# syoyo/lucille

Hardware: AMD Instinct MI355X
Metric: Mrays/s (primary+AO) (higher is better)
Workload: dtype f32 filter + f64 resolve (hit records f64); 1 GPU; S-soup-1M ray dump (BASELINE config 3): 1000000 random triangles, one dump of 100000000 incoherent rays cut into 1 contiguous slice(s), closest-hit; rays=100000000, rays_per_gpu=100000000, triangles=1000000, mode=closest, variant=-1, parallelism=replicated BVH, ray slices x1

## Files before the change

lucille_amd/csrc/lh_device.h:

```cpp
#ifndef LH_DEVICE_H
#define LH_DEVICE_H

#include <stdint.h>
#include <stddef.h>
#include "../../include/lucille_hip.h"

#define LH_BLOCK      256
#define LH_MISS_PRIM  0xFFFFFFFFu
#define LH_T_INF      1.0e38

typedef struct lh_dev_scene {
    const void *nodes;
    const void *tri32;
    const void *tri64;
    float       grid_lo[3], grid_step[3];
    const void *q4nodes;
    uint32_t    nq4nodes, q4_depth;
    uint32_t    q4_stack;
    const void *q8nodes;
    uint32_t    nq8nodes, q8_depth;
    int         prefer_q8;
    uint32_t    stack_rows;
    const void *ref_lca;
    const void *prim_leafpos;
    const void *ref_nodes;
    const void *ref_leaf_prims;
    uint32_t    ref_nnodes;
    int         ref_empty;
    double      ref_bmin[3], ref_bmax[3];
    uint32_t    ntris;
    uint32_t    nnodes;
    uint32_t    max_depth;
    float       scene_r;
    float       deg_dcap;
    uint32_t    cap_srcs;
    uint32_t    ndanger;
    uint32_t    danger[3];
    uint32_t    ray_chunk;
    uint32_t    ray_budget;
    int         stack_guard;
    uint32_t    stack_cap;
    uint32_t    coop_patience;
    uint32_t    ao_group;
    uint32_t    top_nodes;
    uint32_t    io_fmt;
    const void *cam_src;
    const uint32_t *n_dev;
    uint32_t   *diag_out;
    unsigned long long *diag_clock;
} lh_dev_scene_t;

enum { LH_CNT_NODES = 0, LH_CNT_TRIS = 1, LH_CNT_EXACT = 2, LH_CNT_RAYS = 3, LH_CNT_N = 4,
       LH_CNT_NODE_SLOTS = 4, LH_CNT_TRI_SLOTS = 5, LH_CNT_REGROUP_SLOTS = 6,
       LH_CNT_RETRACED = 7,
       LH_CNT_HIST = 8,
       LH_CNT_DEV = 32 };

enum {
    LH_VARIANT_DIRECT = 0,
    LH_VARIANT_SPEC   = 4
};

#define LH_ROWS_UNCHECKED 64u
#define LH_TOP_AUTO       0xFFFFFFFFu
#define LH_TOP_NODES_MAX  512u
#define LH_ROWS_CHECKED   34u
#define LH_NPART          8
#define LH_CURSOR_STRIDE  32
#define LH_CURSOR_WORDS   ((LH_NPART + 1) * LH_CURSOR_STRIDE)
#define LH_AO_QCAP        (1u << 22)
#define LH_DUMP_BUDGET    2048u
#define LH_DUMP_MIN_ACTIVE 24
#define LH_DUMP_TRI_BATCH  8
#define LH_DUMP8_MIN_ACTIVE 40
#define LH_DUMP8_TRI_BATCH  20
#define LH_TILE_CHUNK     1024u
#define LH_AO_BUDGET      384u
#define LH_RAY_BUDGET     128u
#define LH_PRIM_OVERFLOW  0xFFFFFFFDu
#define LH_OCC_OVERFLOW   4u
#define LH_IO_RAYS_F32    1u
#define LH_IO_REC16       2u

#ifdef __cplusplus
extern "C" {
#endif

typedef struct lh_fixq {
    void     *queue;
    uint32_t *qcount;
    uint32_t  qcap;
    void     *aux_stream;
    void     *ev_ready, *ev_done;
} lh_fixq_t;

int lh_launch_trace(const lh_dev_scene_t *sc, size_t n, const double *d_org,
                    const double *d_dir, uint32_t *d_prim, double *d_t,
                    double *d_u, double *d_v, int anyhit, uint8_t *d_occluded,
                    unsigned long long *d_counters ,
                    unsigned long long *d_workq ,
                    int variant, int grid_blocks, int min_active, int tri_batch,
                    const lh_fixq_t *q, int ncus, void *stream);
int lh_launch_trace_ao(const lh_dev_scene_t *sc, size_t nslots, int ntheta, int nphi, unsigned long long seed,
                       const double *d_hitrec, const unsigned long long *d_slot_key, unsigned int *d_occ_count,
                       unsigned long long *d_counters, unsigned long long *d_cursor, int grid_blocks, int min_active,
                       int tri_batch, const lh_fixq_t *q, int ncus, const unsigned long long *d_nslots, uint32_t budget_big, void *stream);
int lh_trace_formats_needed(const lh_dev_scene_t *sc, int variant);
int lh_trace_rows(const lh_dev_scene_t *sc);

// ... 5 lines not shown
```

lucille_amd/csrc/lh_filter.h:

```cpp
#ifndef LH_FILTER_H
#define LH_FILTER_H

#include <math.h>
#include <stdint.h>

#if defined(__HIPCC__)
#define LH_HD __host__ __device__ __forceinline__
#else
#define LH_HD static inline
#endif

#if defined(__HIP_DEVICE_COMPILE__)
#define LH_RCP(a) __builtin_amdgcn_rcpf(a)
#else
#define LH_RCP(a) (1.0f / (a))
#endif

#define LH_EPS24 5.9604645e-8f
#define LH_KBOX  16.0f
#define LH_KTRI  32.0f

typedef struct lh_ray32 {
    float ox, oy, oz, dx, dy, dz;
    float ix, iy, iz;
// ... 29 lines not shown
LH_HD void lh_ray_setup(lh_ray32_t *r, double ox, double oy, double oz,
                        double dx, double dy, double dz, float scene_r)
{
    float omax, scale, pe, sx, sy, sz;
    r->ox = (float)ox; r->oy = (float)oy; r->oz = (float)oz;
    r->dx = (float)dx; r->dy = (float)dy; r->dz = (float)dz;
    r->ix = 1.0f / lh_safe_dir(r->dx);
    r->iy = 1.0f / lh_safe_dir(r->dy);
    r->iz = 1.0f / lh_safe_dir(r->dz);
    omax = fmaxf(fabsf(r->ox), fmaxf(fabsf(r->oy), fabsf(r->oz)));
    scale = omax + scene_r;
    pe = LH_KBOX * LH_EPS24 * scale;
    sx = pe * fabsf(r->ix); sy = pe * fabsf(r->iy); sz = pe * fabsf(r->iz);
    r->cnx = fmaf(-r->ox, r->ix, -sx); r->cfx = fmaf(-r->ox, r->ix, sx);
    r->cny = fmaf(-r->oy, r->iy, -sy); r->cfy = fmaf(-r->oy, r->iy, sy);
    r->cnz = fmaf(-r->oz, r->iz, -sz); r->cfz = fmaf(-r->oz, r->iz, sz);
    r->ngx = r->dx < 0.0f; r->ngy = r->dy < 0.0f; r->ngz = r->dz < 0.0f;
    r->keps = LH_KTRI * LH_EPS24 * scale;
    r->qax = r->qay = r->qaz = 0.0f; r->qbnx = r->qbny = r->qbnz = 0.0f; r->qbfx = r->qbfy = r->qbfz = 0.0f;
    r->dn = sqrtf(fmaf(r->dx, r->dx, fmaf(r->dy, r->dy, r->dz * r->dz))) * 1.000001f;
}

LH_HD int lh_slab(const lh_ray32_t *r, float lox, float loy, float loz,
                  float hix, float hiy, float hiz, float tb, float *tn_out)
{
    const float ax = r->ngx ? hix : lox, bx = r->ngx ? lox : hix;
    const float ay = r->ngy ? hiy : loy, by = r->ngy ? loy : hiy;
    const float az = r->ngz ? hiz : loz, bz = r->ngz ? loz : hiz;
    const float tn = fmaxf(fmaxf(fmaf(ax, r->ix, r->cnx), fmaf(ay, r->iy, r->cny)),
                           fmaxf(fmaf(az, r->iz, r->cnz), 0.0f));
    const float tf = fminf(fminf(fmaf(bx, r->ix, r->cfx), fmaf(by, r->iy, r->cfy)),
                           fminf(fmaf(bz, r->iz, r->cfz), tb));
    *tn_out = tn;
    return tn <= tf;
}

LH_HD int lh_slab_w(const lh_ray32_t *r, uint32_t wx, uint32_t wy, uint32_t wz, float tb, float *tn_out)
{
    const uint32_t sx = r->ngx ? ((wx >> 16) | (wx << 16)) : wx;
    const uint32_t sy = r->ngy ? ((wy >> 16) | (wy << 16)) : wy;
    const uint32_t sz = r->ngz ? ((wz >> 16) | (wz << 16)) : wz;
    const float tn = fmaxf(fmaxf(fmaf((float)(sx & 0xffffu), r->qax, r->qbnx), fmaf((float)(sy & 0xffffu), r->qay, r->qbny)),
                           fmaxf(fmaf((float)(sz & 0xffffu), r->qaz, r->qbnz), 0.0f));
    const float tf = fminf(fminf(fmaf((float)(sx >> 16), r->qax, r->qbfx), fmaf((float)(sy >> 16), r->qay, r->qbfy)),
                           fminf(fmaf((float)(sz >> 16), r->qaz, r->qbfz), tb));
    *tn_out = tn;
    return tn <= tf;
}

#define LH_TRI_REJECT    0
#define LH_TRI_CANDIDATE 1
#define LH_TRI_CERTAIN   2

LH_HD int lh_tri_filter(const lh_ray32_t *r, float v0x, float v0y, float v0z,
                        float e1x, float e1y, float e1z, float e2x, float e2y, float e2z,
                        float ne1, float ne2, float tb, float *t_hi)
{
    const float px = fmaf(r->dy, e2z, -(r->dz * e2y));
    const float py = fmaf(r->dz, e2x, -(r->dx * e2z));
    const float pz = fmaf(r->dx, e2y, -(r->dy * e2x));
    const float a = fmaf(e1x, px, fmaf(e1y, py, e1z * pz));
    const float inva = LH_RCP(a);
    const float sx = r->ox - v0x, sy = r->oy - v0y, sz = r->oz - v0z;
    const float qx = fmaf(sy, e1z, -(sz * e1y));
    const float qy = fmaf(sz, e1x, -(sx * e1z));
    const float qz = fmaf(sx, e1y, -(sy * e1x));
    const float u = fmaf(sx, px, fmaf(sy, py, sz * pz)) * inva;
    const float v = fmaf(qx, r->dx, fmaf(qy, r->dy, qz * r->dz)) * inva;
    const float t = fmaf(e2x, qx, fmaf(e2y, qy, e2z * qz)) * inva;
    const float g = r->keps * fabsf(inva);
    const float tolu = g * r->dn * ne2, tolv = g * r->dn * ne1, tolt = g * ne1 * ne2;
    const float rela = (LH_KTRI * LH_EPS24) * ne1 * ne2 * r->dn * fabsf(inva);
    if (!(rela < 0.5f)) { *t_hi = 3.0e38f; return LH_TRI_CANDIDATE; }
    const int reject = (u < -tolu) | (u > 1.0f + tolu) | (v < -tolv) |
                       (u + v > 1.0f + tolu + tolv) | (t < -tolt) | (t - tolt > tb);
    if (reject) return LH_TRI_REJECT;
    {
        const int sure = (u >= tolu) & (u <= 1.0f - tolu) & (v >= tolv) &
                         (u + v <= 1.0f - tolu - tolv) & (t >= tolt) & (rela < 0.25f) &
                         (fabsf(a) > 2.0e-14f) & (t + tolt < 1.0e37f);
        *t_hi = (t + tolt) * 1.000001f;
        return sure ? LH_TRI_CERTAIN : LH_TRI_CANDIDATE;
    }
}

#if defined(__clang__)
#define LH_NO_CONTRACT _Pragma("clang fp contract(off)")
#else
#define LH_NO_CONTRACT
#endif

LH_HD int lh_exact_isect(const double *tv, double ox, double oy, double oz,
                         double dx, double dy, double dz,
                         double *t_out, double *u_out, double *v_out)
{
    LH_NO_CONTRACT
    const double v0x = tv[0], v0y = tv[1], v0z = tv[2];
    const double e1x = tv[3] - v0x, e1y = tv[4] - v0y, e1z = tv[5] - v0z;
    const double e2x = tv[6] - v0x, e2y = tv[7] - v0y, e2z = tv[8] - v0z;
    const double px = dy * e2z - dz * e2y;
    const double py = dz * e2x - dx * e2z;
    const double pz = dx * e2y - dy * e2x;
    const double a = e1x * px + e1y * py + e1z * pz;
    double inva, sx, sy, sz, qx, qy, qz, u, v, t;
    if (!(fabs(a) > 1.0e-14)) return 0;
    inva = 1.0 / a;
    sx = ox - v0x; sy = oy - v0y; sz = oz - v0z;
    qx = sy * e1z - sz * e1y;
    qy = sz * e1x - sx * e1z;
    qz = sx * e1y - sy * e1x;
    u = (sx * px + sy * py + sz * pz) * inva;
    v = (qx * dx + qy * dy + qz * dz) * inva;
    t = (e2x * qx + e2y * qy + e2z * qz) * inva;
    if ((u < 0.0) || (u > 1.0)) return 0;
    if ((v < 0.0) || ((u + v) > 1.0)) return 0;
    if (t < 0.0) return 0;
    *t_out = t; *u_out = u; *v_out = v;
    return 1;
}

#endif
```

lucille_amd/csrc/lh_kernels.hip:

```cpp
#include <hip/hip_runtime.h>
#include <stdint.h>
#include <string.h>
#include <stdlib.h>
#include <pthread.h>

#include "../../include/lucille_hip.h"
#include "lh_device.h"
#include "lh_filter.h"
#include "lh_reftrace.h"
#include "lh_ao.h"

namespace {

#include "lh_walk.h"
#include "lh_pt.h"

template <bool ANYHIT, bool COUNT>
__device__ __forceinline__ void traverse(Lane &L, const lh_dev_scene_t &sc,
                                         int (*stk)[LH_BLOCK], const int tid,
                                         double ox, double oy, double oz,
                                         double dx, double dy, double dz, Best &best,
                                         uint32_t &c_nodes, uint32_t &c_tris, uint32_t &c_exact)
{
    const float4 *__restrict__ tris  = (const float4 *)sc.tri32;
// ... 62 lines not shown
    const int base = L.sp + nh - 1;
    if (SORTED) {
        const uint32_t k0 = h0 ? ((__float_as_uint(t0) & ~3u) | 0u) : 0xFFFFFFFCu;
        const uint32_t k1 = h1 ? ((__float_as_uint(t1) & ~3u) | 1u) : 0xFFFFFFFDu;
        const uint32_t k2 = h2 ? ((__float_as_uint(t2) & ~3u) | 2u) : 0xFFFFFFFEu;
        const uint32_t k3 = h3 ? ((__float_as_uint(t3) & ~3u) | 3u) : 0xFFFFFFFFu;
        const int b10 = k1 < k0, b20 = k2 < k0, b30 = k3 < k0, b21 = k2 < k1, b31 = k3 < k1, b32 = k3 < k2;
        const int rk0 = b10 + b20 + b30, rk1 = (1 - b10) + b21 + b31;
        const int rk2 = (2 - b20 - b21) + b32, rk3 = 3 - b30 - b31 - b32;
        stk[LH_ROW(h0 ? base - rk0 : L.sp + rk0)][tid] = (int)r.x;
        stk[LH_ROW(h1 ? base - rk1 : L.sp + rk1)][tid] = (int)r.y;
        stk[LH_ROW(h2 ? base - rk2 : L.sp + rk2)][tid] = (int)r.z;
        stk[LH_ROW(h3 ? base - rk3 : L.sp + rk3)][tid] = (int)r.w;
    } else {
        const int a1 = (int)h0, a2 = a1 + (int)h1, a3 = a2 + (int)h2;
        stk[LH_ROW(h0 ? base : base + 1)][tid] = (int)r.x;
        stk[LH_ROW(h1 ? base - a1 : base + 1)][tid] = (int)r.y;
        stk[LH_ROW(h2 ? base - a2 : base + 1)][tid] = (int)r.z;
        stk[LH_ROW(h3 ? base - a3 : base + 1)][tid] = (int)r.w;
    }
    L.sp = base;
    const int nxt = stk[LH_ROW(base)][tid];
    const int popped2 = stk[LH_ROW(L.sp - 1)][tid];
    const bool is_leaf = (nxt < 0) & (nxt != kDone);
    const bool park = is_leaf & (pend == kNoLeaf);
    pend = park ? nxt : pend;
    L.cur = park ? popped2 : nxt;
    L.sp -= park ? 1 : 0;
}

template <bool ANYHIT, bool COUNT, int STRIDE, bool RING>
__device__ __forceinline__ void tri_pass(Lane &L, int &pend, const lh_dev_scene_t &sc, int (*stk)[STRIDE], const int tid,
                                         double ox, double oy, double oz, double dx, double dy, double dz, Best &best,
                                         uint32_t &c_tris, uint32_t &c_exact, const int ring_mask = 0)
{
    if (pend != kNoLeaf) {
        const float4 *__restrict__ tris = (const float4 *)sc.tri32;
        const uint32_t x = ~(uint32_t)pend;
        const float4 *tp = tris + 3 * (size_t)(x >> 2);
        const float4 ta = tp[0], tb_ = tp[1], tc = tp[2];
        if (COUNT) c_tris++;
        const bool finished = tri_step<ANYHIT, COUNT>(L, sc, ta.x, ta.y, ta.z, ta.w, tb_.x, tb_.y, tb_.z, tb_.w, tc.x, tc.z, tc.w, __float_as_uint(tc.y), ox, oy, oz, dx, dy, dz, best, c_exact);
        if (finished) { L.cur = kDone; pend = kNoLeaf; }
        else if (x & 3u) pend = (int)~(((x >> 2) + 1u) << 2 | ((x & 3u) - 1u));
        else {
            const bool waiting = (L.cur < 0) & (L.cur != kDone);
            pend = waiting ? L.cur : kNoLeaf;
            if (waiting) { L.sp--; L.cur = stk[LH_ROW(L.sp)][tid]; }
        }
    }
#undef LH_ROW
}

template <bool ANYHIT, bool COUNT, bool GUARD, bool SORTED = true>
__device__ __forceinline__ void traverse_spec4(Lane &L, int &pend, const lh_dev_scene_t &sc,
                                               int (*stk)[LH_BLOCK], const int tid,
                                               double ox, double oy, double oz,
                                               double dx, double dy, double dz, Best &best,
                                               uint32_t &c_nodes, uint32_t &c_tris, uint32_t &c_exact,
                                               const int min_active, const int tri_batch,
                                               uint32_t &c_nslots, uint32_t &c_tslots, uint32_t &it)
{
    const int rows = (int)sc.stack_rows;
    const uint4 *top = (const uint4 *)(&stk[rows][0]);
    const uint32_t ntop = sc.top_nodes;
    for (;;) {
        if (COUNT) { if (__ballot(L.cur >= 0) != 0ull) c_nslots++; }
        if (GUARD) {
            const bool ov = (L.cur >= 0) & (L.sp + 4 > rows);
            if (__builtin_expect(__ballot(ov) != 0ull, 0)) { if (ov) { L.over = true; L.cur = kDone; pend = kNoLeaf; } }
        }
        if (L.cur >= 0) node_step4<COUNT, LH_BLOCK, false, SORTED>(L, pend, sc, stk, tid, c_nodes, 0, top, ntop);
        const unsigned long long m_node = __ballot(L.cur >= 0);
        const unsigned long long m_pend = __ballot(pend != kNoLeaf);
        if (m_pend != 0ull && (__popcll(m_pend) >= tri_batch || m_node == 0ull)) {
            if (COUNT) c_tslots++;
            tri_pass<ANYHIT, COUNT, LH_BLOCK, false>(L, pend, sc, stk, tid, ox, oy, oz, dx, dy, dz, best, c_tris, c_exact);
        }
        const unsigned long long m_work = __ballot((L.cur != kDone) | (pend != kNoLeaf));
        if (__popcll(m_work) < min_active || (++it & kRegroupMask) == 0u) break;
    }
}

template <bool ANYHIT, bool COUNT>
__device__ __forceinline__ void traverse_spec8(Lane &L, int &pend, const lh_dev_scene_t &sc,
                                               int (*stk)[LH_BLOCK], const int tid,
                                               double ox, double oy, double oz,
                                               double dx, double dy, double dz, Best &best,
                                               uint32_t &c_nodes, uint32_t &c_tris, uint32_t &c_exact,
                                               const int min_active, const int tri_batch,
                                               uint32_t &c_nslots, uint32_t &c_tslots, uint32_t &it)
{
    const float4 *__restrict__ tris  = (const float4 *)sc.tri32;
    const uint32_t oct = (uint32_t)L.r.ngx | ((uint32_t)L.r.ngy << 1) | ((uint32_t)L.r.ngz << 2);
    const int rows = (int)sc.stack_rows - 1;

    for (;;) {
        if (COUNT) { if (__ballot(L.cur >= 0) != 0ull) c_nslots++; }
        if (sc.stack_guard && L.cur >= 0 && L.sp + 8 > rows) { L.over = true; L.cur = kDone; pend = kNoLeaf; }
        if (L.cur >= 0) {
            const uint4 *p = (const uint4 *)sc.q8nodes + 8 * (size_t)L.cur;
            const uint4 a = p[0], b = p[1], c = p[2], d = p[3], e = p[4], f = p[5], r0 = p[6], r1 = p[7];
            if (COUNT) c_nodes++;
            float t;
            const bool h0 = slab_w(L, a.x, a.y, a.z, t) & ((int)r0.x != kDone);
            const bool h1 = slab_w(L, a.w, b.x, b.y, t) & ((int)r0.y != kDone);
            const bool h2 = slab_w(L, b.z, b.w, c.x, t) & ((int)r0.z != kDone);
            const bool h3 = slab_w(L, c.y, c.z, c.w, t) & ((int)r0.w != kDone);
            const bool h4 = slab_w(L, d.x, d.y, d.z, t) & ((int)r1.x != kDone);
            const bool h5 = slab_w(L, d.w, e.x, e.y, t) & ((int)r1.y != kDone);
            const bool h6 = slab_w(L, e.z, e.w, f.x, t) & ((int)r1.z != kDone);
            const bool h7 = slab_w(L, f.y, f.z, f.w, t) & ((int)r1.w != kDone);
            const uint32_t pm = ((uint32_t)h0 << (0u ^ oct)) | ((uint32_t)h1 << (1u ^ oct)) | ((uint32_t)h2 << (2u ^ oct)) |
                                ((uint32_t)h3 << (3u ^ oct)) | ((uint32_t)h4 << (4u ^ oct)) | ((uint32_t)h5 << (5u ^ oct)) |
                                ((uint32_t)h6 << (6u ^ oct)) | ((uint32_t)h7 << (7u ^ oct));
            const int base = L.sp + __popc(pm) - 1;
#define LH_PUSH8(S, H, REF) stk[(H) ? base - __popc(pm & ((1u << ((S) ^ oct)) - 1u)) : rows][tid] = (int)(REF)
            LH_PUSH8(0u, h0, r0.x); LH_PUSH8(1u, h1, r0.y); LH_PUSH8(2u, h2, r0.z); LH_PUSH8(3u, h3, r0.w);
            LH_PUSH8(4u, h4, r1.x); LH_PUSH8(5u, h5, r1.y); LH_PUSH8(6u, h6, r1.z); LH_PUSH8(7u, h7, r1.w);
#undef LH_PUSH8
            L.sp = base;
            const int nxt = stk[base][tid];
            const int popped2 = stk[L.sp - 1][tid];
            const bool is_leaf = (nxt < 0) & (nxt != kDone);
            const bool park = is_leaf & (pend == kNoLeaf);
            pend = park ? nxt : pend;
            L.cur = park ? popped2 : nxt;
            L.sp -= park ? 1 : 0;
        }
        const unsigned long long m_node = __ballot(L.cur >= 0);
        const unsigned long long m_pend = __ballot(pend != kNoLeaf);
        if (m_pend != 0ull && (__popcll(m_pend) >= tri_batch || m_node == 0ull)) {
            if (COUNT) c_tslots++;
            if (pend != kNoLeaf) {
                const uint32_t x = ~(uint32_t)pend;
                const float4 *tp = tris + 3 * (size_t)(x >> 2);
                const float4 ta = tp[0], tb_ = tp[1], tc = tp[2];
                if (COUNT) c_tris++;
                const bool finished = tri_step<ANYHIT, COUNT>(L, sc, ta.x, ta.y, ta.z, ta.w, tb_.x, tb_.y, tb_.z, tb_.w, tc.x, tc.z, tc.w, __float_as_uint(tc.y), ox, oy, oz, dx, dy, dz, best, c_exact);
                if (finished) { L.cur = kDone; pend = kNoLeaf; }
                else if (x & 3u) pend = (int)~(((x >> 2) + 1u) << 2 | ((x & 3u) - 1u));
                else {
                    const bool waiting = (L.cur < 0) & (L.cur != kDone);
                    pend = waiting ? L.cur : kNoLeaf;
                    if (waiting) { L.sp--; L.cur = stk[L.sp][tid]; }
                }
            }
        }
        const unsigned long long m_work = __ballot((L.cur != kDone) | (pend != kNoLeaf));
        if (__popcll(m_work) < min_active || (++it & kRegroupMask) == 0u) break;
    }
}


template <bool IO = true>
__device__ __forceinline__ void dump_ray(const lh_dev_scene_t &sc, size_t i, const double *__restrict__ org, const double *__restrict__ dir,
                                         double &ox, double &oy, double &oz, double &dx, double &dy, double &dz)
{
    if (IO && (sc.io_fmt & LH_IO_RAYS_F32)) {
        const float *o = (const float *)org + 3 * i, *d = (const float *)dir + 3 * i;
        ox = (double)o[0]; oy = (double)o[1]; oz = (double)o[2];
        dx = (double)d[0]; dy = (double)d[1]; dz = (double)d[2];
    } else {
        ox = org[3 * i]; oy = org[3 * i + 1]; oz = org[3 * i + 2];
        dx = dir[3 * i]; dy = dir[3 * i + 1]; dz = dir[3 * i + 2];
    }
}

template <bool FMT = true>
__device__ __forceinline__ uint32_t &rec_prim(const lh_dev_scene_t &sc, uint32_t *prim, size_t i)
{
    return prim[(FMT && (sc.io_fmt & LH_IO_REC16)) ? 4 * i : i];
}

template <bool FMT = true>
__device__ __forceinline__ void store_rec(const lh_dev_scene_t &sc, size_t i, uint32_t *__restrict__ prim, double *__restrict__ t,
                                          double *__restrict__ u, double *__restrict__ v, uint32_t p, double tt, double uu, double vv)
{
    if (FMT && (sc.io_fmt & LH_IO_REC16)) {
        uint4 r;
        r.x = p; r.y = __float_as_uint((float)tt); r.z = __float_as_uint((float)uu); r.w = __float_as_uint((float)vv);
        ((uint4 *)prim)[i] = r;
    } else {
        prim[i] = p; t[i] = tt; u[i] = uu; v[i] = vv;
    }
// ... 181 lines not shown
                    uint32_t chunk = sc.ray_chunk;
                    if ((SRC != 1 && sc.n_dev) || (SRC == 1 && ao.nslots_dev)) {
                        const uint32_t c = n / (gridDim.x * (LH_BLOCK / 64) * 4u);
                        chunk = c < 64u ? 64u : (c < chunk ? c : chunk);
                    }
                    for (;;) {
                        if (drained == (1u << LH_NPART) - 1u) {
                            exhausted = true;
    #ifdef LH_DIAG_CLOCK
                            if (sc.diag_clock && (tid & 63) == 0) sc.diag_clock[(size_t)(2 * gridDim.x + blockIdx.x) * (LH_BLOCK / 64) + (tid >> 6)] = wall_clock64();
    #endif
                            break;
                        }
                        if (drained & (1u << part)) { part = (part + 1u) % LH_NPART; continue; }
                        const uint32_t p0 = per * part, p1 = (p0 + per < n) ? p0 + per : n;
                        const uint32_t plen = p1 > p0 ? p1 - p0 : 0u;
                        uint32_t b = plen;
                        if (plen) {
                            if ((tid & 63) == 0) b = atomicAdd(cursor + part * LH_CURSOR_STRIDE, chunk);
                            b = (uint32_t)__shfl((int)b, 0);
                        }
                        if (b < plen) { b += p0; wbase = b; wend = (p1 - b > chunk) ? b + chunk : p1; break; }
                        drained |= 1u << part;
                        uint32_t seen = 0;
                        if ((tid & 63) == 0) {
                            seen = __hip_atomic_load(cursor + LH_NPART * LH_CURSOR_STRIDE, __ATOMIC_RELAXED, __HIP_MEMORY_SCOPE_AGENT);
                            if ((seen & drained) != drained) atomicOr(cursor + LH_NPART * LH_CURSOR_STRIDE, drained);
                        }
                        drained |= (uint32_t)__shfl((int)seen, 0);
                        part = (part + 1u) % LH_NPART;
                    }
                }
                if (!exhausted) {
                    const uint32_t avail = wend - wbase;
                    const int take = avail < (uint32_t)(need - filled) ? (int)avail : need - filled;
                    if (idle && rank >= filled && rank < filled + take) newray = wbase + (uint32_t)(rank - filled);
                    wbase += (uint32_t)take; filled += take;
                }
            }
        }
        if (newray != kNoRay) {
            const uint32_t i = newray;
            my = i;
            src_ray<SRC, IO>(sc, i, org, dir, ao, ox, oy, oz, dx, dy, dz, selfp);
            lane_init(L, sc, ox, oy, oz, dx, dy, dz);
            best.t = LH_T_INF; best.u = 0.0; best.v = 0.0; best.prim = LH_MISS_PRIM; best.frag = 0u;
            stk[0][tid] = kDone;
            if ((SRC == 0 ? (sc.cap_srcs & 1u) != 0u : sc.deg_dcap < 1.0f) && __builtin_expect(ray_needs_ref_walk(sc, L, dx, dy, dz), 0)) LH_FORCE_REF_WALK(L, best);
            it0 = it;
        }
        const unsigned long long work = __ballot((L.cur != kDone) | (pend != 0));
        if (work == 0ull) break;
        const int thresh = exhausted ? 1 : min_active;
        if (WALK == 3)
            traverse_spec4<ANYHIT, COUNT, false, !(ANYHIT && LH_AO_UNSORTED)>(L, pend, sc, stk, tid, ox, oy, oz, dx, dy, dz, best, cn, ct, ce, thresh, tri_batch, cns, cts, it);
        else if (WALK == 8)
            traverse_spec4<ANYHIT, COUNT, true, !(ANYHIT && LH_AO_UNSORTED)>(L, pend, sc, stk, tid, ox, oy, oz, dx, dy, dz, best, cn, ct, ce, thresh, tri_batch, cns, cts, it);
        else
            traverse_spec8<ANYHIT, COUNT>(L, pend, sc, stk, tid, ox, oy, oz, dx, dy, dz, best, cn, ct, ce, thresh, tri_batch, cns, cts, it);
    }
#ifdef LH_DIAG_CLOCK
    if (sc.diag_clock && (tid & 63) == 0) sc.diag_clock[(size_t)(gridDim.x + blockIdx.x) * (LH_BLOCK / 64) + (tid >> 6)] = wall_clock64();
#endif
    if ((tid & 63) == 0) __hip_atomic_fetch_add(fq.qcount + 2, 1u, __ATOMIC_RELEASE, __HIP_MEMORY_SCOPE_AGENT);
    if (COUNT) {
        add_counters(counters, cn, ct, ce, cr);
        atomicAdd(&counters[LH_CNT_NODE_SLOTS], (unsigned long long)cns);
        atomicAdd(&counters[LH_CNT_TRI_SLOTS], (unsigned long long)cts);
        atomicAdd(&counters[LH_CNT_REGROUP_SLOTS], (unsigned long long)crs);
    }
}

template <bool ANYHIT, bool COUNT, int WALK, int SRC, bool IO = false>
__global__ __launch_bounds__(LH_BLOCK, WALK == 7 ? 3 : 4) void k_trace_persist_lane(
    lh_dev_scene_t sc, uint32_t n, const double *__restrict__ org, const double *__restrict__ dir,
    uint32_t *__restrict__ prim, double *__restrict__ t, double *__restrict__ u,
    double *__restrict__ v, uint8_t *__restrict__ occ, unsigned long long *counters,
    uint32_t *cursor, int min_active, int tri_batch, const AoSrc ao, const FixQ fq)
{
    extern __shared__ int lh_stack_lds[];
    if (SRC != 1 && sc.n_dev) n = *sc.n_dev;
    if (SRC == 1 && ao.nslots_dev) n = (uint32_t)*ao.nslots_dev * (uint32_t)(ao.ntheta * ao.nphi);
    if (WALK != 7 && sc.top_nodes) {
        uint4 *dst = (uint4 *)(lh_stack_lds + (size_t)sc.stack_rows * LH_BLOCK);
        const uint4 *src = (const uint4 *)sc.q4nodes;
        for (uint32_t k = threadIdx.x; k < sc.top_nodes * 4u; k += LH_BLOCK) dst[k] = src[k];
        __syncthreads();
    }
    trace_persist_lane<ANYHIT, COUNT, WALK, SRC, IO>(sc, n, org, dir, prim, t, u, v, occ, counters, cursor, min_active, tri_batch, ao, fq, lh_stack_lds);
}

#define LH_COOP_ROWS_MAX 272

__device__ __forceinline__ void merge_best(const lh_dev_scene_t &sc, Best &g, const Best &b, double dx, double dy, double dz)
{
    if (b.prim == LH_MISS_PRIM) return;
    if (g.prim == LH_MISS_PRIM) { g = b; return; }
    bool take = b.t < g.t;
    if (!take && b.t == g.t && b.prim != g.prim) take = tie_takes_new(sc, b.prim, g.prim, dx, dy, dz);
    const double tm = fabs(b.t) > fabs(g.t) ? fabs(b.t) : fabs(g.t);
    const uint32_t near2 = (b.prim != g.prim && b.t != g.t && fabs(b.t - g.t) <= LH_FRAGILE_REL * tm) ? 2u : 0u;
    const uint32_t sticky = ((g.frag | b.frag) & 2u) | near2;
    if (take) { g.t = b.t; g.u = b.u; g.v = b.v; g.prim = b.prim; g.frag = b.frag & 1u; }
    g.frag = (g.frag & 1u) | sticky;
}

struct RefHit { double t, u, v; uint32_t prim; };
__device__ __noinline__ RefHit ref_trace_one(const lh_dev_scene_t &sc, double ox, double oy, double oz, double dx, double dy, double dz)
{
    RefHit h; uint32_t p = LH_MISS_PRIM; double tt = LH_T_INF, uu = 0.0, vv = 0.0;
    const int hit = lh_ref_trace((const lh_refnode_t *)sc.ref_nodes, (const uint32_t *)sc.ref_leaf_prims, (const double *)sc.tri64,
                                 sc.ref_empty, sc.ref_bmin, sc.ref_bmax, ox, oy, oz, dx, dy, dz, &p, &tt, &uu, &vv);
// ... 576 lines not shown
```

lucille_amd/csrc/lh_query.hip:

```cpp
#include <atomic>
#include <chrono>
#include <condition_variable>
#include <deque>
#include <mutex>
#include <thread>
#include <vector>

#include "lh_internal.h"

__global__ void k_fill_miss(size_t n, uint32_t *prim, double *t, double *u, double *v, uint8_t *occ, uint4 *rec16)
{
    size_t i = (size_t)blockIdx.x * blockDim.x + threadIdx.x;
    if (i >= n) return;
    if (rec16) { uint4 r; r.x = LH_MISS_PRIM; r.y = __float_as_uint((float)LH_T_INF); r.z = r.w = __float_as_uint(0.0f); rec16[i] = r; }
    if (prim) prim[i] = LH_MISS_PRIM;
    if (t) t[i] = LH_T_INF;
    if (u) u[i] = 0.0;
    if (v) v[i] = 0.0;
    if (occ) occ[i] = 0;
}

int lh_aoq_slot(lh_accel_t *a, hipStream_t s)
{
    int k, free_k = -1;
// ... 91 lines not shown
    if (lh_ensure_formats(a, lh_trace_formats_needed(&a->dev, variant)) != 0) return -1;
    const bool q8 = dump && dump_walks_q8(a, variant);
    if (q8 && lh_ensure_formats(a, LH_FMT_Q8) != 0) return -1;
    const int qk = lh_aoq_slot(a, s);
    if (qk < 0) return -1;
    lh_dev_scene_t sc = a->dev;
    sc.prefer_q8 = q8;
    if (dump) sc.ray_budget = a->dump_budget;
    else if (sc.ray_chunk < LH_TILE_CHUNK) sc.ray_chunk = LH_TILE_CHUNK;
    sc.io_fmt = opt.io_fmt & (mode == LH_MODE_ANY ? LH_IO_RAYS_F32 : (LH_IO_RAYS_F32 | LH_IO_REC16));
    sc.diag_out = opt.diag_out; sc.n_dev = opt.n_dev; sc.cam_src = opt.cam_src; sc.diag_clock = opt.diag_clock;
    const bool dump4 = dump && !q8 && !a->knobs_user;
    const bool dump8 = dump && q8 && !a->knobs_user;
    int rc = lh_launch_trace(&sc, n, (const double *)d_org, (const double *)d_dir, (uint32_t *)d_prim,
                             (double *)d_t, (double *)d_u, (double *)d_v, mode == LH_MODE_ANY,
                             (uint8_t *)d_occ, d_counters, (unsigned long long *)((uint32_t *)a->d_cursor + (size_t)LH_CURSOR_WORDS * (a->cursor_next++ % LH_NCURSOR)), variant, a->grid_blocks,
                             dump4 ? LH_DUMP_MIN_ACTIVE : dump8 ? LH_DUMP8_MIN_ACTIVE : a->min_active, dump4 ? LH_DUMP_TRI_BATCH : dump8 ? LH_DUMP8_TRI_BATCH : a->tri_batch,
                             &a->aoq[qk].q, a->ncus, (void *)s);
    if (rc != 0) return fail("kernel launch failed: %s", hipGetErrorString(hipGetLastError()));
    return 0;
}

extern "C" int lh_accel_intersect_device(lh_accel_t *a, size_t n, const void *d_org, const void *d_dir,
                                         void *d_prim, void *d_t, void *d_u, void *d_v, void *d_occ,
                                         int mode, int variant, void *stream)
{
    lh_guard guard(a);
    return lh_launch(a, n, d_org, d_dir, d_prim, d_t, d_u, d_v, d_occ, mode, variant, NULL, (hipStream_t)stream, true);
}

extern "C" int lh_accel_intersect_device_counted(lh_accel_t *a, size_t n, const void *d_org, const void *d_dir,
                                                 void *d_prim, void *d_t, void *d_u, void *d_v, void *d_occ,
                                                 int mode, int variant, uint64_t counters[4])
{
    lh_guard guard(a);
    if (!a || !a->committed) return fail("intersect: accel not committed");
    if (!counters) return fail("intersect_counted: counters is NULL");
    HIPCHK(hipSetDevice(a->device));
    HIPCHK(hipMemsetAsync(a->d_counters, 0, sizeof(unsigned long long) * LH_CNT_DEV, a->stream));
    HIPCHK(hipDeviceSynchronize());
    if (a->hs->bvh.ntris == 0) { counters[0] = counters[1] = counters[2] = 0; counters[3] = n; }
    int rc = lh_launch(a, n, d_org, d_dir, d_prim, d_t, d_u, d_v, d_occ, mode, variant, a->d_counters, a->stream, true);
    if (rc != 0) return rc;
    HIPCHK(hipStreamSynchronize(a->stream));
    if (a->hs->bvh.ntris) {
        unsigned long long h[LH_CNT_DEV];
        HIPCHK(hipMemcpy(h, a->d_counters, sizeof(h), hipMemcpyDeviceToHost));
        for (int k = 0; k < LH_CNT_N; k++) counters[k] = h[k];
        a->last_retraced = h[LH_CNT_RETRACED];
        if (getenv("LH_DEBUG_COUNTERS"))
            fprintf(stderr, "[lucille_hip] lane slots: node steps %llu of %llu, triangle steps %llu of %llu, regroup iterations %llu; "
                            "rays through the reference walk %llu\n",
                    h[LH_CNT_NODES], h[LH_CNT_NODE_SLOTS], h[LH_CNT_TRIS], h[LH_CNT_TRI_SLOTS], h[LH_CNT_REGROUP_SLOTS], h[LH_CNT_RETRACED]);
    }
    return 0;
}

extern "C" int lh_accel_dump_node_bytes(const lh_accel_t *a)
{
    if (!a || !a->committed || a->hs->bvh.ntris == 0) return 0;
    return dump_walks_q8(a, a->default_variant) ? (int)sizeof(lh_q8node_t) : 64;
}

extern "C" uint64_t lh_accel_last_retraced(const lh_accel_t *a) { return a ? a->last_retraced : 0; }

int lh_ensure_stage(lh_accel_t *a, size_t bytes)
{
    if (a->stage_bytes >= bytes) return 0;
    if (a->d_stage) { (void)hipFree(a->d_stage); a->d_stage = NULL; a->stage_bytes = 0; }
    HIPCHK(hipMalloc(&a->d_stage, bytes));
    a->stage_bytes = bytes;
    return 0;
}

#define LH_PIPE_CHUNK_DEFAULT ((size_t)1 << 21)
#define LH_PIPE_DEPTH_DEFAULT 3
#define LH_PIPE_MIN   ((size_t)1 << 21)
#define LH_COPY_SLICE ((size_t)1 << 20)

namespace {
struct CopyJob { char *dst; const char *src; size_t bytes; std::atomic<size_t> *left; };
struct CopyPool {
    std::mutex mu; std::condition_variable cv;
    std::deque<CopyJob> q;
    int nthreads;
};
CopyPool *g_pool;
std::once_flag g_pool_once;

bool pool_take(CopyPool *P, CopyJob &j, bool wait)
{
    std::unique_lock<std::mutex> lk(P->mu);
    if (wait) P->cv.wait(lk, [&] { return !P->q.empty(); });
    if (P->q.empty()) return false;
    j = P->q.front(); P->q.pop_front();
    return true;
}

void pool_worker(CopyPool *P)
{
    for (;;) {
        CopyJob j;
        pool_take(P, j, true);
        memcpy(j.dst, j.src, j.bytes);
        j.left->fetch_sub(1, std::memory_order_release);
    }
// ... 663 lines not shown
```

lucille_amd/csrc/lh_walk.h:

```cpp
#ifndef LH_WALK_H
#define LH_WALK_H

constexpr int   kDone  = (int)0x80000000;
constexpr int   kPend  = 4;

struct Best {
    double   t, u, v;
    uint32_t prim;
    uint32_t frag;
};

__device__ __noinline__ bool tie_takes_new(const lh_dev_scene_t &sc, uint32_t pnew, uint32_t pold,
                                           double dx, double dy, double dz)
{
    if (!sc.ref_lca) return pnew > pold;
    const uint2 *lp = (const uint2 *)sc.prim_leafpos;
    const int4 *nd = (const int4 *)sc.ref_lca;
    const uint2 a = lp[pnew], b = lp[pold];
    if (a.x == b.x) return a.y > b.y;
    int ca = (int)a.x, cb = (int)b.x;
    int4 na = nd[ca], nb = nd[cb];
    while (na.y > nb.y) { ca = na.x; na = nd[ca]; }
    while (nb.y > na.y) { cb = nb.x; nb = nd[cb]; }
    while (na.x != nb.x) { ca = na.x; na = nd[ca]; cb = nb.x; nb = nd[cb]; }
// ... 20 lines not shown
    }
}

struct Lane {
    lh_ray32_t r;
    uint32_t sh[3];
    float tb;
    int   cur, sp;
    uint32_t p0, p1, p2, p3;
    int   np;
    bool  certain;
    bool  over;
};

__device__ __forceinline__ void lane_init(Lane &L, const lh_dev_scene_t &sc,
                                          double ox, double oy, double oz,
                                          double dx, double dy, double dz)
{
    lh_ray_setup(&L.r, ox, oy, oz, dx, dy, dz, sc.scene_r);
    lh_ray_setup_grid(&L.r, sc.grid_lo, sc.grid_step, sc.scene_r);
    L.sh[0] = L.r.ngx ? 16u : 0u; L.sh[1] = L.r.ngy ? 16u : 0u; L.sh[2] = L.r.ngz ? 16u : 0u;
    L.tb = 1.0e38f;
    L.cur = 0; L.sp = 1;
    L.p0 = L.p1 = L.p2 = L.p3 = LH_MISS_PRIM; L.np = 0;
    L.certain = false; L.over = false;
}


__device__ __forceinline__ bool slab_w(const Lane &L, uint32_t wx, uint32_t wy, uint32_t wz, float &tn_out);
__device__ __forceinline__ bool ray_needs_ref_walk(const lh_dev_scene_t &sc, const Lane &L, double dx, double dy, double dz)
{
    const double D = fmax(fabs(dx), fmax(fabs(dy), fabs(dz)));
    if (!((D > (double)sc.deg_dcap) & (sc.ref_nodes != NULL))) return false;
    if (sc.ndanger == LH_DANGER_ALL || D > LH_DEG_DCAP_ALL) return true;
    float tn;
    return slab_w(L, sc.danger[0], sc.danger[1], sc.danger[2], tn);
}
#define LH_FORCE_REF_WALK(L, best) do { (L).tb = -1.0f; (best).prim = 0u; (best).frag = 1u; } while (0)

__device__ __forceinline__ bool slab_w(const Lane &L, uint32_t wx, uint32_t wy, uint32_t wz, float &tn_out)
{
    const uint32_t sx = __builtin_amdgcn_alignbit(wx, wx, L.sh[0]);
    const uint32_t sy = __builtin_amdgcn_alignbit(wy, wy, L.sh[1]);
    const uint32_t sz = __builtin_amdgcn_alignbit(wz, wz, L.sh[2]);
    const float tn = fmaxf(fmaxf(fmaf((float)(sx & 0xffffu), L.r.qax, L.r.qbnx), fmaf((float)(sy & 0xffffu), L.r.qay, L.r.qbny)),
                           fmaxf(fmaf((float)(sz & 0xffffu), L.r.qaz, L.r.qbnz), 0.0f));
    const float tf = fminf(fminf(fmaf((float)(sx >> 16), L.r.qax, L.r.qbfx), fmaf((float)(sy >> 16), L.r.qay, L.r.qbfy)),
                           fminf(fmaf((float)(sz >> 16), L.r.qaz, L.r.qbfz), L.tb));
    tn_out = tn;
    return tn <= tf;
}

template <bool ANYHIT, bool COUNT, class RayLoad>
__device__ __forceinline__ bool tri_step_g(Lane &L, const lh_dev_scene_t &sc, float v0x, float v0y, float v0z,
                                           float e1x, float e1y, float e1z, float e2x, float e2y, float e2z,
                                           float ne1, float ne2, uint32_t prim, RayLoad ray, Best &best, uint32_t &c_exact)
{
    float t_hi;
    const int cls = lh_tri_filter(&L.r, v0x, v0y, v0z, e1x, e1y, e1z, e2x, e2y, e2z, ne1, ne2, L.tb, &t_hi);
    if (cls == LH_TRI_REJECT) return false;
    const bool sure = (cls == LH_TRI_CERTAIN);
    if (ANYHIT && sure) { L.certain = true; return true; }
    if (sure) L.tb = fminf(L.tb, t_hi);
    if (L.np == kPend) {
        if (COUNT) c_exact += kPend;
        double ox, oy, oz, dx, dy, dz;
        ray(ox, oy, oz, dx, dy, dz);
        resolve(sc, L.p0, ox, oy, oz, dx, dy, dz, best);
        resolve(sc, L.p1, ox, oy, oz, dx, dy, dz, best);
        resolve(sc, L.p2, ox, oy, oz, dx, dy, dz, best);
        resolve(sc, L.p3, ox, oy, oz, dx, dy, dz, best);
        L.np = 0;
        if (ANYHIT && best.prim != LH_MISS_PRIM) return true;
    }
    L.p3 = L.p2; L.p2 = L.p1; L.p1 = L.p0; L.p0 = prim; L.np++;
    return false;
}

template <bool ANYHIT, bool COUNT>
__device__ __forceinline__ bool tri_step(Lane &L, const lh_dev_scene_t &sc, float v0x, float v0y, float v0z,
                                         float e1x, float e1y, float e1z, float e2x, float e2y, float e2z,
                                         float ne1, float ne2, uint32_t prim,
                                         double ox, double oy, double oz, double dx, double dy, double dz,
                                         Best &best, uint32_t &c_exact)
{
    return tri_step_g<ANYHIT, COUNT>(L, sc, v0x, v0y, v0z, e1x, e1y, e1z, e2x, e2y, e2z, ne1, ne2, prim,
                                     [=](double &a, double &b, double &c, double &d, double &e, double &f) { a = ox; b = oy; c = oz; d = dx; e = dy; f = dz; },
                                     best, c_exact);
}

template <bool ANYHIT, bool COUNT>
__device__ __forceinline__ void finish(Lane &L, const lh_dev_scene_t &sc,
                                       double ox, double oy, double oz,
                                       double dx, double dy, double dz, Best &best,
                                       uint32_t &c_exact, const uint32_t skip = LH_MISS_PRIM)
{
    if (ANYHIT && (L.certain || best.prim != LH_MISS_PRIM)) return;
    if (L.np > 0 && L.p0 != skip) { if (COUNT) c_exact++; resolve(sc, L.p0, ox, oy, oz, dx, dy, dz, best); }
    if (L.np > 1 && L.p1 != skip) { if (COUNT) c_exact++; resolve(sc, L.p1, ox, oy, oz, dx, dy, dz, best); }
    if (L.np > 2 && L.p2 != skip) { if (COUNT) c_exact++; resolve(sc, L.p2, ox, oy, oz, dx, dy, dz, best); }
    if (L.np > 3 && L.p3 != skip) { if (COUNT) c_exact++; resolve(sc, L.p3, ox, oy, oz, dx, dy, dz, best); }
    L.np = 0;
}

#endif
```

Baseline: 2283 Mrays/s.

## Add cooperative wavefront leaf pass that spreads parked leaf triangles across lanes

Adds a cooperative leaf pass for the SRC==0 trace path. Each lane's parked leaf triangles, plus a second leaf it is waiting on, are compacted across the 64-lane wavefront with ds_permute. Every lane then runs the f32 triangle classify for one item using the owner's ray fetched by bpermute, and the results are shuffled back so the owners book them in order. The triangle filter is split into classify and a t-cull step so the cull can use the owner's current tb. The goal is to keep more lanes busy during triangle tests on incoherent rays. The cost is extra cross-lane permutes, ballot loops and register pressure, and the t-cull runs against tb values that may be stale.

```diff
diff --git a/lucille_amd/csrc/lh_device.h b/lucille_amd/csrc/lh_device.h
--- a/lucille_amd/csrc/lh_device.h
+++ b/lucille_amd/csrc/lh_device.h
@@ -54,7 +54,8 @@
        LH_CNT_NODE_SLOTS = 4, LH_CNT_TRI_SLOTS = 5, LH_CNT_REGROUP_SLOTS = 6,
        LH_CNT_RETRACED = 7,
        LH_CNT_HIST = 8,
-       LH_CNT_DEV = 32 };
+       LH_CNT_LEAF_HIST = 32,
+       LH_CNT_DEV = 36 };
 
 enum {
     LH_VARIANT_DIRECT = 0,
diff --git a/lucille_amd/csrc/lh_filter.h b/lucille_amd/csrc/lh_filter.h
--- a/lucille_amd/csrc/lh_filter.h
+++ b/lucille_amd/csrc/lh_filter.h
@@ -105,9 +105,9 @@
 #define LH_TRI_CANDIDATE 1
 #define LH_TRI_CERTAIN   2
 
-LH_HD int lh_tri_filter(const lh_ray32_t *r, float v0x, float v0y, float v0z,
-                        float e1x, float e1y, float e1z, float e2x, float e2y, float e2z,
-                        float ne1, float ne2, float tb, float *t_hi)
+LH_HD int lh_tri_classify(const lh_ray32_t *r, float v0x, float v0y, float v0z,
+                          float e1x, float e1y, float e1z, float e2x, float e2y, float e2z,
+                          float ne1, float ne2, float *t_lo, float *t_hi)
 {
     const float px = fmaf(r->dy, e2z, -(r->dz * e2y));
     const float py = fmaf(r->dz, e2x, -(r->dx * e2z));
@@ -124,17 +124,33 @@
     const float g = r->keps * fabsf(inva);
     const float tolu = g * r->dn * ne2, tolv = g * r->dn * ne1, tolt = g * ne1 * ne2;
     const float rela = (LH_KTRI * LH_EPS24) * ne1 * ne2 * r->dn * fabsf(inva);
-    if (!(rela < 0.5f)) { *t_hi = 3.0e38f; return LH_TRI_CANDIDATE; }
-    const int reject = (u < -tolu) | (u > 1.0f + tolu) | (v < -tolv) |
-                       (u + v > 1.0f + tolu + tolv) | (t < -tolt) | (t - tolt > tb);
-    if (reject) return LH_TRI_REJECT;
+    if (!(rela < 0.5f)) { *t_lo = -INFINITY; *t_hi = 3.0e38f; return LH_TRI_CANDIDATE; }
+    *t_lo = t - tolt;
+    *t_hi = (t + tolt) * 1.000001f;
     {
+        const int reject = (u < -tolu) | (u > 1.0f + tolu) | (v < -tolv) |
+                           (u + v > 1.0f + tolu + tolv) | (t < -tolt);
         const int sure = (u >= tolu) & (u <= 1.0f - tolu) & (v >= tolv) &
                          (u + v <= 1.0f - tolu - tolv) & (t >= tolt) & (rela < 0.25f) &
                          (fabsf(a) > 2.0e-14f) & (t + tolt < 1.0e37f);
-        *t_hi = (t + tolt) * 1.000001f;
-        return sure ? LH_TRI_CERTAIN : LH_TRI_CANDIDATE;
+        return reject ? LH_TRI_REJECT : (sure ? LH_TRI_CERTAIN : LH_TRI_CANDIDATE);
     }
+}
+
+LH_HD int lh_tri_cull(float t_lo, float tb)
+{
+    return t_lo > tb;
+}
+
+LH_HD int lh_tri_filter(const lh_ray32_t *r, float v0x, float v0y, float v0z,
+                        float e1x, float e1y, float e1z, float e2x, float e2y, float e2z,
+                        float ne1, float ne2, float tb, float *t_hi)
+{
+    float lo, hi;
+    const int cls = lh_tri_classify(r, v0x, v0y, v0z, e1x, e1y, e1z, e2x, e2y, e2z, ne1, ne2, &lo, &hi);
+    if (cls == LH_TRI_REJECT || lh_tri_cull(lo, tb)) return LH_TRI_REJECT;
+    *t_hi = hi;
+    return cls;
 }
 
 #if defined(__clang__)
diff --git a/lucille_amd/csrc/lh_kernels.hip b/lucille_amd/csrc/lh_kernels.hip
--- a/lucille_amd/csrc/lh_kernels.hip
+++ b/lucille_amd/csrc/lh_kernels.hip
@@ -138,14 +138,99 @@
 #undef LH_ROW
 }
 
-template <bool ANYHIT, bool COUNT, bool GUARD, bool SORTED = true>
+constexpr uint32_t kItemReject = 0xFFFFFFFFu;
+
+__device__ __forceinline__ uint32_t lanes_below(const unsigned long long m)
+{
+    return __builtin_amdgcn_mbcnt_hi((uint32_t)(m >> 32), __builtin_amdgcn_mbcnt_lo((uint32_t)m, 0u));
+}
+__device__ __forceinline__ uint32_t pull_u(const uint32_t src_lane, const uint32_t x) { return (uint32_t)__builtin_amdgcn_ds_bpermute((int)(src_lane << 2), (int)x); }
+__device__ __forceinline__ float pull_f(const uint32_t src_lane, const float x) { return __int_as_float(__builtin_amdgcn_ds_bpermute((int)(src_lane << 2), __float_as_int(x))); }
+
+template <bool ANYHIT, bool COUNT>
+__device__ __forceinline__ void leaf_pass_coop(Lane &L, int &pend, const lh_dev_scene_t &sc, int (*stk)[LH_BLOCK], const int tid,
+                                               double ox, double oy, double oz, double dx, double dy, double dz, Best &best,
+                                               uint32_t &c_tris, uint32_t &c_exact, unsigned long long *counters)
+{
+    const uint32_t lane = (uint32_t)tid & 63u;
+    const bool parked = pend != kNoLeaf;
+    const bool waiting = parked & (L.cur < 0) & (L.cur != kDone);
+    const uint32_t cnt = (parked ? (~(uint32_t)pend & 3u) + 1u : 0u) + (waiting ? (~(uint32_t)L.cur & 3u) + 1u : 0u);
+
+    uint32_t item = 0u, off = 0u;
+#pragma nounroll
+    for (uint32_t k = 0; k < 8u; k++) {
+        const unsigned long long bk = __ballot(cnt > k);
+        if (bk == 0ull || off >= 64u) break;
+        const uint32_t nk = (uint32_t)__popcll(bk), room = 64u - off, nw = nk < room ? nk : room;
+        const uint32_t rank = lanes_below(bk);
+        const bool writer = (cnt > k) & (rank < nw);
+        const uint32_t rest = lane - (rank < nw ? rank : nw);
+        const uint32_t dst = writer ? off + rank : (rest < off ? rest : rest + nw);
+        const uint32_t got = (uint32_t)__builtin_amdgcn_ds_permute((int)(dst << 2), (int)(lane | (k << 8)));
+        item = (lane >= off) & (lane < off + nw) ? got : item;
+        off += nw;
+    }
+    const bool has_item = lane < off;
+    const uint32_t owner = has_item ? (item & 63u) : lane, k_mine = has_item ? item >> 8 : 0u;
+
+    uint32_t word = kItemReject; float t_lo = 0.0f, t_hi = 0.0f;
+    {
+        const uint32_t xp = ~pull_u(owner, (uint32_t)pend), xc = ~pull_u(owner, (uint32_t)L.cur);
+        const uint32_t c1 = (xp & 3u) + 1u;
+        const uint32_t tri = k_mine < c1 ? (xp >> 2) + k_mine : (xc >> 2) + (k_mine - c1);
+        lh_ray32_t fr;
+        fr.ox = pull_f(owner, L.r.ox); fr.oy = pull_f(owner, L.r.oy); fr.oz = pull_f(owner, L.r.oz);
+        fr.dx = pull_f(owner, L.r.dx); fr.dy = pull_f(owner, L.r.dy); fr.dz = pull_f(owner, L.r.dz);
+        fr.keps = pull_f(owner, L.r.keps); fr.dn = pull_f(owner, L.r.dn);
+        if (has_item) {
+            const float4 *tp = (const float4 *)sc.tri32 + 3 * (size_t)tri;
+            const float4 ta = tp[0], tb_ = tp[1], tc = tp[2];
+            const int cls = lh_tri_classify(&fr, ta.x, ta.y, ta.z, ta.w, tb_.x, tb_.y, tb_.z, tb_.w, tc.x, tc.z, tc.w, &t_lo, &t_hi);
+            if (cls != LH_TRI_REJECT) word = __float_as_uint(tc.y) | ((uint32_t)cls << 30);
+        }
+    }
+
+    bool live = parked;
+    off = 0u;
+#pragma nounroll
+    for (uint32_t k = 0; k < 8u; k++) {
+        const unsigned long long bk = __ballot(cnt > k);
+        if (bk == 0ull || off >= 64u) break;
+        const uint32_t nk = (uint32_t)__popcll(bk), room = 64u - off, nw = nk < room ? nk : room;
+        const uint32_t rank = lanes_below(bk);
+        const bool mine = (cnt > k) & (rank < nw);
+        const uint32_t src = mine ? off + rank : lane;
+        const uint32_t w = pull_u(src, word);
+        const float lo = pull_f(src, t_lo), hi = pull_f(src, t_hi);
+        if (mine & live) {
+            if (COUNT) c_tris++;
+            bool finished = false;
+            if (w != kItemReject && !lh_tri_cull(lo, L.tb))
+                finished = tri_book_g<ANYHIT, COUNT>(L, sc, (int)(w >> 30), hi, w & 0x3FFFFFFFu,
+                                                     [=](double &a, double &b, double &c, double &d, double &e, double &f) { a = ox; b = oy; c = oz; d = dx; e = dy; f = dz; },
+                                                     best, c_exact);
+            const uint32_t x = ~(uint32_t)pend;
+            if (finished) { L.cur = kDone; pend = kNoLeaf; live = false; }
+            else if (x & 3u) pend = (int)~(((x >> 2) + 1u) << 2 | ((x & 3u) - 1u));
+            else {
+                const bool second = (L.cur < 0) & (L.cur != kDone);
+                pend = second ? L.cur : kNoLeaf;
+                if (second) { L.sp--; L.cur = stk[L.sp][tid]; if (COUNT) atomicAdd(&counters[LH_CNT_LEAF_HIST + (~(uint32_t)pend & 3u)], 1ull); }
+            }
+        }
+        off += nw;
+    }
+}
+
+template <bool ANYHIT, bool COUNT, bool GUARD, bool SORTED = true, bool COOP = false>
 __device__ __forceinline__ void traverse_spec4(Lane &L, int &pend, const lh_dev_scene_t &sc,
                                                int (*stk)[LH_BLOCK], const int tid,
                                                double ox, double oy, double oz,
                                                double dx, double dy, double dz, Best &best,
                                                uint32_t &c_nodes, uint32_t &c_tris, uint32_t &c_exact,
                                                const int min_active, const int tri_batch,
-                                               uint32_t &c_nslots, uint32_t &c_tslots, uint32_t &it)
+                                               uint32_t &c_nslots, uint32_t &c_tslots, uint32_t &it, unsigned long long *counters = NULL)
 {
     const int rows = (int)sc.stack_rows;
     const uint4 *top = (const uint4 *)(&stk[rows][0]);
@@ -156,10 +241,18 @@
             const bool ov = (L.cur >= 0) & (L.sp + 4 > rows);
             if (__builtin_expect(__ballot(ov) != 0ull, 0)) { if (ov) { L.over = true; L.cur = kDone; pend = kNoLeaf; } }
         }
+        const int pend0 = pend;
         if (L.cur >= 0) node_step4<COUNT, LH_BLOCK, false, SORTED>(L, pend, sc, stk, tid, c_nodes, 0, top, ntop);
+        if (COUNT && COOP && pend != pend0) atomicAdd(&counters[LH_CNT_LEAF_HIST + (~(uint32_t)pend & 3u)], 1ull);
         const unsigned long long m_node = __ballot(L.cur >= 0);
         const unsigned long long m_pend = __ballot(pend != kNoLeaf);
-        if (m_pend != 0ull && (__popcll(m_pend) >= tri_batch || m_node == 0ull)) {
+        if (COOP) {
+            const unsigned long long m_wait = __ballot(L.cur != kDone) & ~m_node;
+            if (m_pend != 0ull && (__popcll(m_pend) + __popcll(m_wait) >= tri_batch || m_node == 0ull)) {
+                if (COUNT) c_tslots++;
+                leaf_pass_coop<ANYHIT, COUNT>(L, pend, sc, stk, tid, ox, oy, oz, dx, dy, dz, best, c_tris, c_exact, counters);
+            }
+        } else if (m_pend != 0ull && (__popcll(m_pend) >= tri_batch || m_node == 0ull)) {
             if (COUNT) c_tslots++;
             tri_pass<ANYHIT, COUNT, LH_BLOCK, false>(L, pend, sc, stk, tid, ox, oy, oz, dx, dy, dz, best, c_tris, c_exact);
         }
@@ -168,14 +261,14 @@
     }
 }
 
-template <bool ANYHIT, bool COUNT>
+template <bool ANYHIT, bool COUNT, bool COOP = false>
 __device__ __forceinline__ void traverse_spec8(Lane &L, int &pend, const lh_dev_scene_t &sc,
                                                int (*stk)[LH_BLOCK], const int tid,
                                                double ox, double oy, double oz,
                                                double dx, double dy, double dz, Best &best,
                                                uint32_t &c_nodes, uint32_t &c_tris, uint32_t &c_exact,
                                                const int min_active, const int tri_batch,
-                                               uint32_t &c_nslots, uint32_t &c_tslots, uint32_t &it)
+                                               uint32_t &c_nslots, uint32_t &c_tslots, uint32_t &it, unsigned long long *counters = NULL)
 {
     const float4 *__restrict__ tris  = (const float4 *)sc.tri32;
     const uint32_t oct = (uint32_t)L.r.ngx | ((uint32_t)L.r.ngy << 1) | ((uint32_t)L.r.ngz << 2);
@@ -184,6 +277,7 @@
     for (;;) {
         if (COUNT) { if (__ballot(L.cur >= 0) != 0ull) c_nslots++; }
         if (sc.stack_guard && L.cur >= 0 && L.sp + 8 > rows) { L.over = true; L.cur = kDone; pend = kNoLeaf; }
+        const int pend0 = pend;
         if (L.cur >= 0) {
             const uint4 *p = (const uint4 *)sc.q8nodes + 8 * (size_t)L.cur;
             const uint4 a = p[0], b = p[1], c = p[2], d = p[3], e = p[4], f = p[5], r0 = p[6], r1 = p[7];
@@ -214,9 +308,16 @@
             L.cur = park ? popped2 : nxt;
             L.sp -= park ? 1 : 0;
         }
+        if (COUNT && COOP && pend != pend0) atomicAdd(&counters[LH_CNT_LEAF_HIST + (~(uint32_t)pend & 3u)], 1ull);
         const unsigned long long m_node = __ballot(L.cur >= 0);
         const unsigned long long m_pend = __ballot(pend != kNoLeaf);
-        if (m_pend != 0ull && (__popcll(m_pend) >= tri_batch || m_node == 0ull)) {
+        if (COOP) {
+            const unsigned long long m_wait = __ballot(L.cur != kDone) & ~m_node;
+            if (m_pend != 0ull && (__popcll(m_pend) + __popcll(m_wait) >= tri_batch || m_node == 0ull)) {
+                if (COUNT) c_tslots++;
+                leaf_pass_coop<ANYHIT, COUNT>(L, pend, sc, stk, tid, ox, oy, oz, dx, dy, dz, best, c_tris, c_exact, counters);
+            }
+        } else if (m_pend != 0ull && (__popcll(m_pend) >= tri_batch || m_node == 0ull)) {
             if (COUNT) c_tslots++;
             if (pend != kNoLeaf) {
                 const uint32_t x = ~(uint32_t)pend;
@@ -504,12 +605,13 @@
         const unsigned long long work = __ballot((L.cur != kDone) | (pend != 0));
         if (work == 0ull) break;
         const int thresh = exhausted ? 1 : min_active;
+        constexpr bool COOP = (SRC == 0);
         if (WALK == 3)
-            traverse_spec4<ANYHIT, COUNT, false, !(ANYHIT && LH_AO_UNSORTED)>(L, pend, sc, stk, tid, ox, oy, oz, dx, dy, dz, best, cn, ct, ce, thresh, tri_batch, cns, cts, it);
+            traverse_spec4<ANYHIT, COUNT, false, !(ANYHIT && LH_AO_UNSORTED), COOP>(L, pend, sc, stk, tid, ox, oy, oz, dx, dy, dz, best, cn, ct, ce, thresh, tri_batch, cns, cts, it, counters);
         else if (WALK == 8)
-            traverse_spec4<ANYHIT, COUNT, true, !(ANYHIT && LH_AO_UNSORTED)>(L, pend, sc, stk, tid, ox, oy, oz, dx, dy, dz, best, cn, ct, ce, thresh, tri_batch, cns, cts, it);
+            traverse_spec4<ANYHIT, COUNT, true, !(ANYHIT && LH_AO_UNSORTED), COOP>(L, pend, sc, stk, tid, ox, oy, oz, dx, dy, dz, best, cn, ct, ce, thresh, tri_batch, cns, cts, it, counters);
         else
-            traverse_spec8<ANYHIT, COUNT>(L, pend, sc, stk, tid, ox, oy, oz, dx, dy, dz, best, cn, ct, ce, thresh, tri_batch, cns, cts, it);
+            traverse_spec8<ANYHIT, COUNT, COOP>(L, pend, sc, stk, tid, ox, oy, oz, dx, dy, dz, best, cn, ct, ce, thresh, tri_batch, cns, cts, it, counters);
     }
 #ifdef LH_DIAG_CLOCK
     if (sc.diag_clock && (tid & 63) == 0) sc.diag_clock[(size_t)(gridDim.x + blockIdx.x) * (LH_BLOCK / 64) + (tid >> 6)] = wall_clock64();
diff --git a/lucille_amd/csrc/lh_query.hip b/lucille_amd/csrc/lh_query.hip
--- a/lucille_amd/csrc/lh_query.hip
+++ b/lucille_amd/csrc/lh_query.hip
@@ -167,6 +167,9 @@
             fprintf(stderr, "[lucille_hip] lane slots: node steps %llu of %llu, triangle steps %llu of %llu, regroup iterations %llu; "
                             "rays through the reference walk %llu\n",
                     h[LH_CNT_NODES], h[LH_CNT_NODE_SLOTS], h[LH_CNT_TRIS], h[LH_CNT_TRI_SLOTS], h[LH_CNT_REGROUP_SLOTS], h[LH_CNT_RETRACED]);
+        if (getenv("LH_DEBUG_COUNTERS"))
+            fprintf(stderr, "[lucille_hip] visited leaves of 1 / 2 / 3 / 4 triangles: %llu %llu %llu %llu\n",
+                    h[LH_CNT_LEAF_HIST], h[LH_CNT_LEAF_HIST + 1], h[LH_CNT_LEAF_HIST + 2], h[LH_CNT_LEAF_HIST + 3]);
     }
     return 0;
 }
diff --git a/lucille_amd/csrc/lh_walk.h b/lucille_amd/csrc/lh_walk.h
--- a/lucille_amd/csrc/lh_walk.h
+++ b/lucille_amd/csrc/lh_walk.h
@@ -96,13 +96,9 @@
 }
 
 template <bool ANYHIT, bool COUNT, class RayLoad>
-__device__ __forceinline__ bool tri_step_g(Lane &L, const lh_dev_scene_t &sc, float v0x, float v0y, float v0z,
-                                           float e1x, float e1y, float e1z, float e2x, float e2y, float e2z,
-                                           float ne1, float ne2, uint32_t prim, RayLoad ray, Best &best, uint32_t &c_exact)
+__device__ __forceinline__ bool tri_book_g(Lane &L, const lh_dev_scene_t &sc, const int cls, const float t_hi, uint32_t prim,
+                                           RayLoad ray, Best &best, uint32_t &c_exact)
 {
-    float t_hi;
-    const int cls = lh_tri_filter(&L.r, v0x, v0y, v0z, e1x, e1y, e1z, e2x, e2y, e2z, ne1, ne2, L.tb, &t_hi);
-    if (cls == LH_TRI_REJECT) return false;
     const bool sure = (cls == LH_TRI_CERTAIN);
     if (ANYHIT && sure) { L.certain = true; return true; }
     if (sure) L.tb = fminf(L.tb, t_hi);
@@ -119,6 +115,17 @@
     }
     L.p3 = L.p2; L.p2 = L.p1; L.p1 = L.p0; L.p0 = prim; L.np++;
     return false;
+}
+
+template <bool ANYHIT, bool COUNT, class RayLoad>
+__device__ __forceinline__ bool tri_step_g(Lane &L, const lh_dev_scene_t &sc, float v0x, float v0y, float v0z,
+                                           float e1x, float e1y, float e1z, float e2x, float e2y, float e2z,
+                                           float ne1, float ne2, uint32_t prim, RayLoad ray, Best &best, uint32_t &c_exact)
+{
+    float t_hi;
+    const int cls = lh_tri_filter(&L.r, v0x, v0y, v0z, e1x, e1y, e1z, e2x, e2y, e2z, ne1, ne2, L.tb, &t_hi);
+    if (cls == LH_TRI_REJECT) return false;
+    return tri_book_g<ANYHIT, COUNT>(L, sc, cls, t_hi, prim, ray, best, c_exact);
 }
 
 template <bool ANYHIT, bool COUNT>
```

After: 2001 Mrays/s. -12.3%, worse.
